# jianwen-xie/Latent-Space-Normalizing-Flow

Hardware: AMD Instinct MI355X
Metric: latent-samples/sec through flow+logdet, nz=128 B=65536 (higher is better)
Workload: dtype bf16x3; 1 GPU; CIFAR-10 flow prior nz=128 f_width=64 f_depth=5 affine, forward+logdet+log-prob, B=65536 synthetic z per evaluation (BASELINE.json configs[2]); rows_per_gpu=65536, global_rows=65536, parallelism=single GPU, streams=3, clock_ramp_launches_before_warmup=600

## Files before the change

### latent-space-normalizing-flow_amd/csrc/lsnf_fwd3p.hip

```cpp
#include <stdlib.h>
#include <type_traits>
#include "lsnf_l16.h"

#if LSNF_L16_PARTS != 3
#error "lsnf_fwd3p.hip is the three-term bf16 kernel"
#endif

#ifndef LSNF_FILLMASK
#define LSNF_FILLMASK 0x7f
#endif

namespace {

struct Fwd3pArgs {
    const float* consts; const float* panels3;
    const float* z_in; const float* objective;
    float* z_out; float* logdet_out; float* ll_out;
    int B, nz, half, n_blocks, vec4;
    double* stats;
    float* hdump; int width;
    float* z_saved; float* act_saved;
    unsigned long long* stamps;
};

#ifdef LSNF_STAMPS
#define P_STAMP(i, INSN)                                                                                \
    do { __builtin_amdgcn_sched_barrier(0);                                                             \
         unsigned long long t_; asm volatile(INSN " %0\n\ts_waitcnt lgkmcnt(0)" : "=s"(t_) :: "memory");  \
         __builtin_amdgcn_sched_barrier(0);                                                             \
         if (a.stamps && lane == 0) a.stamps[(((size_t)blockIdx.x * NWAVES + wave) & 2047) * 64 + (i)] = t_; } while (0)
#else
#define P_STAMP(i, INSN) do {} while (0)
#endif

template <int WT_>
struct Fwd3pCfg : LsnfStackCfg<2, WT_> {
    using S = LsnfStackCfg<2, WT_>;
    static constexpr int F = LSNF_FRAG3_FLOATS;
    static constexpr int OFF3_S2 = F * S::P1 * S::KT1;
    static constexpr int OFF3_S3 = OFF3_S2 + F * S::P2 * S::KT2;
    static constexpr int OFF3_S4 = OFF3_S3 + F * S::P3 * S::KT3;
    static constexpr int BLOCK3 = OFF3_S4 + F * S::P4 * S::KT4;
    static constexpr int SLOT3 = 2 * S::MAXKT * F;
    static constexpr int CONST_FLOATS = S::FWD_CONST;
};

__device__ __forceinline__ void keep(unsigned a, unsigned b, unsigned c) { asm volatile("" :: "v"(a), "v"(b), "v"(c)); }
__device__ __forceinline__ void keep(float a, float b, float c, float d, float e) { asm volatile("" :: "v"(a), "v"(b), "v"(c), "v"(d), "v"(e)); }

struct StepDesc { int acc, tile, s, frag; };
template <int KT> constexpr StepDesc mkstep(int acc, int tl, int in_tile, int kt, int s) { return StepDesc{acc, in_tile, s, ((tl * KT + kt) * 2 + s) * 3}; }

struct Tile16 { f32x4v q[4]; };
struct SplitTile16 { unsigned d[2][3][4]; };

template <int HT, int ST>
__device__ __forceinline__ Tile16 load_tile16(int t, const float* __restrict__ z, const int* rows, int nz, int half, int g, int vw) {
    Tile16 x;
    const int hh = t / HT, tt = t % HT;
#pragma unroll
    for (int ft = 0; ft < 2; ++ft)
#pragma unroll
        for (int st = 0; st < ST; ++st) {
            const int f0 = 32 * tt + l16_feat0(ft, g), col0 = hh * half + f0, q = 2 * ft + st;
            const float* zr = z + (long)rows[st] * (long)nz;
            if (vw == 4) {
                f32x4 v = {0.f, 0.f, 0.f, 0.f};
                if (f0 < half) v = *reinterpret_cast<const f32x4*>(zr + col0);
                x.q[q][0] = v[0]; x.q[q][1] = v[1]; x.q[q][2] = v[2]; x.q[q][3] = v[3];
            } else if (vw == 2) {
                f32x2 v0 = {0.f, 0.f}, v1 = {0.f, 0.f};
                if (f0 < half) v0 = *reinterpret_cast<const f32x2*>(zr + col0);
                if (f0 + 2 < half) v1 = *reinterpret_cast<const f32x2*>(zr + col0 + 2);
                x.q[q][0] = v0[0]; x.q[q][1] = v0[1]; x.q[q][2] = v1[0]; x.q[q][3] = v1[1];
            } else {
#pragma unroll
                for (int j = 0; j < 4; ++j) x.q[q][j] = (f0 + j < half) ? zr[col0 + j] : 0.0f;
            }
        }
    return x;
}
template <int HT, int ST>
__device__ __forceinline__ void store_tile16(int t, const Tile16& x, float* __restrict__ z, const int* rows, const bool* live,
                                             int nz, int half, int g, int vw) {
    const int hh = t / HT, tt = t % HT;
#pragma unroll
    for (int ft = 0; ft < 2; ++ft)
#pragma unroll
        for (int st = 0; st < ST; ++st) {
            if (!live[st]) continue;
            const int f0 = 32 * tt + l16_feat0(ft, g), col0 = hh * half + f0, q = 2 * ft + st;
            float* zr = z + (long)rows[st] * (long)nz;
            if (vw == 4) {
                if (f0 < half) { f32x4 v = {x.q[q][0], x.q[q][1], x.q[q][2], x.q[q][3]}; *reinterpret_cast<f32x4*>(zr + col0) = v; }
            } else if (vw == 2) {
                if (f0 < half) { f32x2 v = {x.q[q][0], x.q[q][1]}; *reinterpret_cast<f32x2*>(zr + col0) = v; }
                if (f0 + 2 < half) { f32x2 v = {x.q[q][2], x.q[q][3]}; *reinterpret_cast<f32x2*>(zr + col0 + 2) = v; }
            } else {
#pragma unroll
                for (int j = 0; j < 4; ++j)
                    if (f0 + j < half) zr[col0 + j] = x.q[q][j];
            }
        }
}
__device__ __forceinline__ const float* bias_lane_ptr(const float* cb, int g) { return cb + (g & 1) * 16 + 4 * (g >> 1); }
__device__ __forceinline__ f32x4v bias_quad(const float* lane_ptr, int float_off) {
    const f32x4 v = *reinterpret_cast<const f32x4*>(lane_ptr + float_off);
    f32x4v r;
#pragma unroll
    for (int j = 0; j < 4; ++j) r[j] = v[j];
    return r;
}
template <class PH> constexpr bool first_touch(int i) {
    for (int j = 0; j < i; ++j)
        if (PH::at(j).acc == PH::at(i).acc && PH::at(j).s == PH::at(i).s) return false;
    return true;
}
template <int ST> __device__ __forceinline__ constexpr int unit_quad(int q) { return ST == 2 ? q : (q & ~1); }
template <int ST> __device__ __forceinline__ constexpr int unit_pair0(int q) { return ST == 2 ? 0 : (q & 1); }
template <int ST> __device__ __forceinline__ constexpr int unit_st(int q) { return ST == 2 ? (q & 1) : 0; }
template <bool RELU, int ST>
__device__ __forceinline__ void split_q16(const Tile16& x, int q, SplitTile16& out) {
#pragma clang fp contract(off)
    const int ft = q >> 1, st = unit_st<ST>(q), qr = unit_quad<ST>(q);
#pragma unroll
    for (int jj = 0; jj < ST; ++jj) {
        const int j = unit_pair0<ST>(q) + jj;
        float a = x.q[qr][2 * j], b = x.q[qr][2 * j + 1];
        if (RELU) { a = fmaxf(a, 0.0f); b = fmaxf(b, 0.0f); }
        const unsigned p1 = pk_bf16(a, b);
        a -= __builtin_bit_cast(float, p1 << 16); b -= __builtin_bit_cast(float, p1 & 0xffff0000u);
        const unsigned p2 = pk_bf16(a, b);
        a -= __builtin_bit_cast(float, p2 << 16); b -= __builtin_bit_cast(float, p2 & 0xffff0000u);
        const int d = 2 * ft + j;
        out.d[st][0][d] = p1; out.d[st][1][d] = p2; out.d[st][2][d] = pk_bf16(a, b);
        keep(out.d[st][0][d], out.d[st][1][d], out.d[st][2][d]);
    }
}
template <int ST>
__device__ __forceinline__ void sigmoid_q16(Tile16& p, int q, float* lsum ) {
    const int st = unit_st<ST>(q), qr = unit_quad<ST>(q), r0 = 2 * unit_pair0<ST>(q);
#pragma unroll
    for (int r = r0; r < r0 + 2 * ST; ++r) {
        float sig, l2;
        lsnf_sigmoid_log2(p.q[qr][r], sig, l2);
        p.q[qr][r] = sig; lsum[st] += l2;
    }
    keep(p.q[qr][r0], p.q[qr][r0 + 1], p.q[qr][r0 + 2 * ST - 2], p.q[qr][r0 + 2 * ST - 1], lsum[st]);
}
template <int ST>
__device__ __forceinline__ void couple_q16(Tile16& v, const Tile16& t, const Tile16& sig, int q) {
    const int qr = unit_quad<ST>(q), r0 = 2 * unit_pair0<ST>(q);
#pragma unroll
    for (int r = r0; r < r0 + 2 * ST; ++r) v.q[qr][r] = (v.q[qr][r] + t.q[qr][r]) * sig.q[qr][r];
}

#ifndef LSNF_STASH_AUX
#define LSNF_STASH_AUX 0
#endif
#ifndef LSNF_STASH_PARTS
#define LSNF_STASH_PARTS 7
#endif
typedef unsigned u32x4s __attribute__((ext_vector_type(4)));
struct StashLane { unsigned zoff, soff, moff, msh, hoff; };
struct StashRsrc { __amdgpu_buffer_rsrc_t r[2]; };
__device__ __forceinline__ StashRsrc stash_rsrc(const float* p, unsigned bytes, unsigned second_off) {
    char* c = reinterpret_cast<char*>(const_cast<float*>(p));
    return StashRsrc{{__builtin_amdgcn_make_buffer_rsrc(c, 0, (int)bytes, 0x00020000),
                      __builtin_amdgcn_make_buffer_rsrc(c + second_off, 0, (int)(bytes > second_off ? bytes - second_off : 0u), 0x00020000)}};
}
template <int HT>
__device__ __forceinline__ void stash_row_quad(const StashRsrc& rs, const StashLane& sl, int t, int q, const Tile16& x, int nz, int half, int g) {
    if constexpr (!(LSNF_STASH_PARTS & 4)) return;
    const int ft = q >> 1, st = q & 1, hh = t / HT, tt = t % HT;
    unsigned off = sl.zoff;
    if (st) off += (unsigned)(16 * nz * 4);
    off = (32 * tt + 16 * ft + 4 * g < half) ? off : 0x80000000u;
    const u32x4s v = __builtin_bit_cast(u32x4s, x.q[q]);
    __builtin_amdgcn_raw_buffer_store_b128(v, rs.r[hh], off + (unsigned)((32 * tt + 16 * ft) * 4), 0, LSNF_STASH_AUX);
}
__device__ __forceinline__ void stash_sigma_quad(const StashRsrc& rs, const StashLane& sl, int t, int q, const Tile16& sg) {
    if constexpr (!(LSNF_STASH_PARTS & 2)) return;
    const int ft = q >> 1, st = q & 1;
    const u32x4s v = __builtin_bit_cast(u32x4s, sg.q[q]);
    __builtin_amdgcn_raw_buffer_store_b128(v, rs.r[t], sl.soff + (unsigned)((2 * ft * 64 + 16 * st) * 16), 0, LSNF_STASH_AUX);
}
__device__ __forceinline__ void mask_q16(const Tile16& h, int q, unsigned (&mk)[2][2]) {
    if constexpr (!(LSNF_STASH_PARTS & 1)) return;
    unsigned m = 0;
#pragma unroll
    for (int r = 3; r >= 0; --r) m = __builtin_amdgcn_alignbit(m, __builtin_bit_cast(unsigned, 0.0f - h.q[q][r]), 31);
    mk[q & 1][q >> 1] = m;
    asm volatile("" :: "v"(m));
}
__device__ __forceinline__ void stash_mask_words(const StashRsrc& rs, const StashLane& sl, int tile, const unsigned (&mk)[2][2]) {
    if constexpr (!(LSNF_STASH_PARTS & 1)) return;
    const unsigned w0 = mk[0][0] | (mk[0][1] << 8), w1 = mk[1][0] | (mk[1][1] << 8);
    unsigned x = ((w0 << 16) | w1) << sl.msh;
    x = lsnf_pair_or32(x);
    __builtin_amdgcn_raw_buffer_store_b32(x >> 16, rs.r[0], sl.moff + (unsigned)(tile * 64 * 4), 0, 0);
    __builtin_amdgcn_raw_buffer_store_b32(x & 0xffffu, rs.r[0], sl.moff + (unsigned)((tile * 64 + 16) * 4), 0, 0);
}
__device__ __forceinline__ void stash_h_quad(const StashRsrc& rs, const StashLane& sl, int t, int q, const Tile16& h, int width) {
    const int ft = q >> 1, st = q & 1;
    f32x4v r;
#pragma unroll
    for (int j = 0; j < 4; ++j) r[j] = fmaxf(h.q[q][j], 0.0f);
    const unsigned off = (32 * t + 16 * ft < width) ? sl.hoff : 0x80000000u;
    __builtin_amdgcn_raw_buffer_store_b128(__builtin_bit_cast(u32x4s, r), rs.r[t], off + (unsigned)((ft * 2 + st) * 1024), 0, LSNF_STASH_AUX);
}

template <int NM, int NV>
__device__ __forceinline__ void pin_mfma() {
    lsnf_static_for<NM>([&](auto mc) {
        constexpr int m = decltype(mc)::value, V = NV / NM + (m < NV % NM ? 1 : 0);
        __builtin_amdgcn_sched_group_barrier(0x008, 1, 0);
        if constexpr (V > 0) __builtin_amdgcn_sched_group_barrier(0x402, V, 0);
    });
}
template <class PH, int ST, class Fill, class Mid>
__device__ __forceinline__ void run_phase16(Tile16* acc, const float* bias_ptr , const SplitTile16* in, const float* lbuf, int lane, Fill&& fill, Mid&& mid) {
    const bf16x8* wp = reinterpret_cast<const bf16x8*>(lbuf) + lane;
    __builtin_amdgcn_sched_barrier(0);
    bf16x8 a[3];
#pragma unroll
    for (int p = 0; p < 3; ++p) a[p] = wp[(PH::at(0).frag + p) * 64];
    f32x4v bq = bias_quad(bias_ptr, 32 * PH::btile(PH::at(0).acc) + 8 * PH::at(0).s);
    __builtin_amdgcn_sched_group_barrier(0x100, 4, 0);
    lsnf_static_for<PH::N>([&](auto ic) {
        constexpr int i = decltype(ic)::value;
        constexpr StepDesc d = PH::at(i);
        mid(ic);
        bf16x8 na[3];
        f32x4v nbq = bq;
#pragma unroll
        for (int p = 0; p < 3; ++p) na[p] = a[p];
        if constexpr (i + 1 < PH::N) {
#pragma unroll
            for (int p = 0; p < 3; ++p) na[p] = wp[(PH::at(i + 1).frag + p) * 64];
            if constexpr (first_touch<PH>(i + 1)) nbq = bias_quad(bias_ptr, 32 * PH::btile(PH::at(i + 1).acc) + 8 * PH::at(i + 1).s);
        }
#ifndef LSNF_ABL_NOFILL
        fill(ic);
#endif
        const SplitTile16& x = in[d.tile];
        constexpr bool first = first_touch<PH>(i);
#define LSNF_Q_MMA(WI, XI) \
        acc[d.acc].q[2 * d.s + 0] = __builtin_amdgcn_mfma_f32_16x16x32_bf16(a[WI], __builtin_bit_cast(bf16x8, u32x4{x.d[0][XI][0], x.d[0][XI][1], x.d[0][XI][2], x.d[0][XI][3]}), (first && WI == 2 && XI == 0) ? bq : acc[d.acc].q[2 * d.s + 0], 0, 0, 0); \
        if constexpr (ST == 2) acc[d.acc].q[2 * d.s + 1] = __builtin_amdgcn_mfma_f32_16x16x32_bf16(a[WI], __builtin_bit_cast(bf16x8, u32x4{x.d[1][XI][0], x.d[1][XI][1], x.d[1][XI][2], x.d[1][XI][3]}), (first && WI == 2 && XI == 0) ? bq : acc[d.acc].q[2 * d.s + 1], 0, 0, 0);
#ifdef LSNF_ABL_NOMFMA
        LSNF_Q_MMA(0, 0)
#else
        LSNF_F3_TERMS(LSNF_Q_MMA)
#endif
#undef LSNF_Q_MMA
        if constexpr (i + 1 < PH::N) __builtin_amdgcn_sched_group_barrier(0x100, first_touch<PH>(i + 1) ? 4 : 3, 0);
        pin_mfma<6 * ST, (PH::valu(i) * ST) / 2>();
        __builtin_amdgcn_sched_barrier(0);
#pragma unroll
        for (int p = 0; p < 3; ++p) a[p] = na[p];
        bq = nbq;
    });
}

struct QhNoStores { static constexpr int stores(int) { return 0; } };
struct QhS1a : QhNoStores {
    static constexpr int N = 16;
    static constexpr int btile(int acc) { return acc; }
    static constexpr StepDesc at(int i) { return mkstep<4>((i >> 1) & 1, (i >> 1) & 1, i >> 2, i >> 2, i & 1); }
    static constexpr int valu(int i) { return i < 2 ? 22 : (i < 6 ? 28 : (i < 8 ? 16 : (i < 12 ? 22 : 0))); }
};
struct QhS1b : QhNoStores {
    static constexpr int N = 16;
    static constexpr int btile(int acc) { return 2 + acc; }
    static constexpr StepDesc at(int i) { return mkstep<4>((i >> 1) & 1, (i >> 1) & 1, i >> 2, i >> 2, i & 1); }
    static constexpr int valu(int i) { return i >= 8 ? 22 : 0; }
};
struct QhS23 : QhNoStores {
    static constexpr int N = 16;
    static constexpr int btile(int acc) { return 4 + acc; }
    static constexpr StepDesc at(int i) {
        if (i < 8) { const int tl = i >> 2, kt = (i >> 1) & 1; return mkstep<2>(tl, tl, kt, kt, i & 1); }
        const int j = i - 8, kt = j >> 2, tl = (j >> 1) & 1;
        return mkstep<2>(2 + tl, 2 + tl, 2 + kt, kt, j & 1);
    }
    static constexpr int valu(int i) { return (i >= 4 && i < 12) ? 26 : (i >= 13 ? 26 : 0); }
};
struct QhS4 : QhNoStores {
    static constexpr int N = 16;
    static constexpr int btile(int acc) { return 8 + (acc == 0 ? 2 : (acc == 1 ? 0 : (acc == 2 ? 3 : 1))); }
    static constexpr int torder(int j) { return j == 0 ? 2 : (j == 1 ? 0 : (j == 2 ? 3 : 1)); }
    static constexpr StepDesc at(int i) { const int kt = i >> 3, j = (i >> 1) & 3; return mkstep<2>(j, torder(j), kt, kt, i & 1); }
    static constexpr int valu(int i) { return i < 4 ? 26 : (i < 9 ? 0 : (i < 12 ? 28 : (i == 12 ? 36 : (i == 13 ? 24 : 22)))); }
};

struct QsS1a : QhS1a {
    static constexpr int valu(int i) { return (i == 6 || i == 7) ? 20 : (i >= 8 && i < 12 ? 23 : QhS1a::valu(i)); }
    static constexpr int stores(int i) { return (i >= 2 && i < 6) ? 1 : ((i == 6 || i == 7) ? 2 : (i >= 8 && i < 12 ? 1 : 0)); }
};
struct QsS1b : QhS1b {
    static constexpr int valu(int i) { return i < 8 ? (i >= 6 ? 1 : 0) : (i < 14 ? 23 : 22); }
    static constexpr int stores(int i) { return (i >= 6 && i < 14) ? 1 : 0; }
};
struct QsS23 : QhS23 {
    static constexpr int valu(int i) { return (i >= 4 && i < 12) ? (i == 8 ? 44 : 34) : (i >= 13 ? 34 : 0); }
    static constexpr int stores(int i) { return i == 8 ? 2 : 0; }
};
struct QsS4 : QhS4 {
    static constexpr int valu(int i) { return i < 4 ? 34 : ((i >= 6 && i < 9) ? 10 + QhS4::valu(i) : QhS4::valu(i)); }
    static constexpr int stores(int i) { return (i >= 6 && i < 9) ? 2 : ((i >= 9 && i < 13) ? 1 : 0); }
};
struct QxS23 : QsS23 {
    static constexpr int valu(int i) { return QsS23::valu(i) + (((i >= 4 && i < 12) || i >= 13) ? 2 : 0); }
    static constexpr int stores(int i) { return QsS23::stores(i) + (((i >= 4 && i < 12) || i >= 13) ? 1 : 0); }
};
struct QxS4 : QsS4 {
    static constexpr int valu(int i) { return QsS4::valu(i) + (i < 4 ? 2 : 0); }
    static constexpr int stores(int i) { return QsS4::stores(i) + (i < 4 ? 1 : 0); }
};
template <class PH> constexpr int stores_after(int last_dma_step) {
    int n = 0;
    for (int i = last_dma_step + 1; i < PH::N; ++i) n += PH::stores(i);
    return n;
}

template <int WT, int NWAVES, int ST, int STASH = 0>
__global__ __launch_bounds__(64 * NWAVES, 1) void lsnf_fwd3q_kernel(const Fwd3pArgs a) {
    static_assert(!STASH || ST == 2, "the stash tile is a wave's 32 rows");
    using TS1a = std::conditional_t<STASH != 0, QsS1a, QhS1a>;
    using TS1b = std::conditional_t<STASH != 0, QsS1b, QhS1b>;
    using TS23 = std::conditional_t<STASH == 2, QxS23, std::conditional_t<STASH != 0, QsS23, QhS23>>;
    using TS4 = std::conditional_t<STASH == 2, QxS4, std::conditional_t<STASH != 0, QsS4, QhS4>>;
    using C = Fwd3pCfg<WT>;
    static_assert(WT == 2, "lsnf_fwd3q_kernel: f_width <= 64 instantiation");
    constexpr int THREADS = 64 * NWAVES;
    constexpr int HT = 2, NZT = 4, F = C::F;
    constexpr int SLOT = C::SLOT3;
    extern __shared__ __attribute__((aligned(16))) float smem[];
    float* cst = smem;
    float* const buf0 = smem + a.n_blocks * C::CONST_FLOATS;
    const int tid = threadIdx.x;
    const int wave = __builtin_amdgcn_readfirstlane(tid >> 6);
    const int lane = tid & 63;
    const int n = lane & 15, g = lane >> 4;
    P_STAMP(0, "s_memtime");
    P_STAMP(50, "s_memrealtime");
    const int n_phases = 4 * a.n_blocks;
    auto phase_src = [&](int k) -> const float* {
        const float* gb = a.panels3 + (size_t)(k >> 2) * C::BLOCK3;
        const int j = k & 3;
        return gb + (j == 0 ? 0 : (j == 1 ? 2 * 4 * F : (j == 2 ? C::OFF3_S2 : C::OFF3_S4)));
    };
    auto sync_issue = [&](int k, auto left) {
#ifdef LSNF_ABL_SKIPSYNC
        if ((LSNF_ABL_SKIPSYNC >> (k & 3)) & 1) return;
#endif
        asm volatile("s_waitcnt vmcnt(%0)" :: "n"(decltype(left)::value) : "memory");
        __syncthreads();
#ifdef LSNF_FWD3Q_BURST_DMA
        if (k + 1 < n_phases) issue_kib<48, NWAVES>(phase_src(k + 1), buf0 + ((k + 1) & 1) * SLOT, wave, lane);
#endif
    };
    constexpr int PER_WAVE = 48 / NWAVES, EVERY = STASH ? 1 : 16 / PER_WAVE, LAST_DMA = (PER_WAVE - 1) * EVERY;
    using Left0 = std::integral_constant<int, 0>;
    using LeftS1a = std::integral_constant<int, stores_after<TS1a>(LAST_DMA)>;
    using LeftS1b = std::integral_constant<int, stores_after<TS1b>(LAST_DMA)>;
    using LeftS23 = std::integral_constant<int, stores_after<TS23>(LAST_DMA) + (STASH == 2 ? 1 : 0)>;
    using LeftS4 = std::integral_constant<int, stores_after<TS4>(LAST_DMA)>;
    const float* dma_src = nullptr; float* dma_dst = nullptr;
    auto dma_arm = [&](int k) {
        dma_src = phase_src(k + 1 < n_phases ? k + 1 : k);
        dma_dst = buf0 + ((k + 1) & 1) * SLOT;
    };
    auto dma_step = [&](auto ic) {
#ifndef LSNF_FWD3Q_BURST_DMA
        constexpr int i = decltype(ic)::value;
        if constexpr (i % EVERY == 0 && i / EVERY < PER_WAVE) issue_piece<NWAVES>(dma_src, dma_dst, i / EVERY, wave, lane);
#endif
    };

    const int wbase = (blockIdx.x * NWAVES + wave) * (16 * ST);
    int sample[2] = {0, 0}, rows[2] = {0, 0}; bool live[2] = {false, false};
#pragma unroll
    for (int st = 0; st < ST; ++st) { sample[st] = wbase + 16 * st + n; live[st] = sample[st] < a.B; rows[st] = live[st] ? sample[st] : a.B - 1; }

    Tile16 v[NZT];
    SplitTile16 xs[NZT];
    Tile16 p1, t1;
    float lsum[2] = {0.0f, 0.0f};
    {
        const Tile16 x0 = load_tile16<HT, ST>(0, a.z_in, rows, a.nz, a.half, g, a.vec4);
        const Tile16 x1 = load_tile16<HT, ST>(1, a.z_in, rows, a.nz, a.half, g, a.vec4);
        v[2] = load_tile16<HT, ST>(2, a.z_in, rows, a.nz, a.half, g, a.vec4);
        v[3] = load_tile16<HT, ST>(3, a.z_in, rows, a.nz, a.half, g, a.vec4);
        __builtin_amdgcn_sched_barrier(0);
        issue_kib<48, NWAVES>(phase_src(0), buf0, wave, lane);
        for (int i = tid; i < a.n_blocks * C::CONST_FLOATS; i += THREADS) cst[i] = a.consts[i];
#pragma unroll
        for (int q = 0; q < 4; ++q) { split_q16<false, ST>(x0, q, xs[0]); split_q16<false, ST>(x1, q, xs[1]); }
        split_q16<false, ST>(v[2], 0, xs[2]); split_q16<false, ST>(v[2], 1, xs[2]);
#pragma unroll
        for (int q = 0; q < 4; ++q)
#pragma unroll
            for (int r = 0; r < 4; ++r) { p1.q[q][r] = 80.0f; t1.q[q][r] = 0.0f; }
    }
    float ell[2];
#pragma unroll
    for (int st = 0; st < 2; ++st) ell[st] = (st < ST && a.objective) ? a.objective[rows[st]] : 0.0f;
    float ss01[2] = {0.0f, 0.0f};
    StashLane sl0 = {0u, 0u, 0u, 0u};
    const LsnfActLayout al = lsnf_act_layout(a.B, HT, WT);
    const unsigned zbytes = (unsigned)a.B * (unsigned)a.nz * 4u, abytes = (unsigned)(al.per_block * 4);
    if constexpr (STASH) {
        const unsigned tile_byte = (unsigned)(wbase >> 5) * (unsigned)(al.per_tile * 4), L = (unsigned)(n + 32 * (g & 1));
        sl0.zoff = ((unsigned)(wbase + n) * (unsigned)a.nz + 4u * g) * 4u;
        sl0.soff = tile_byte + ((unsigned)(g >> 1) * 64u + L) * 16u;
        sl0.moff = tile_byte + (unsigned)(al.mask_off * 4) + L * 4u;
        sl0.msh = 4u * (g >> 1);
        sl0.hoff = (unsigned)(wbase >> 5) * (unsigned)(32 * a.width * 4) + (unsigned)(n * 4 + g) * 16u;
    }
    const LsnfDumpLayout dl = lsnf_dump_layout(a.B, a.nz, a.width);
    const unsigned hbytes = (unsigned)(((size_t)a.B + 31) / 32 * 32 * a.width * 4);
    sync_issue(0, Left0{});
    P_STAMP(1, "s_memtime");

    for (int blk = 0; blk < a.n_blocks; ++blk) {
        const float* cb = cst + blk * C::CONST_FLOATS;
        const bool more = blk + 1 < a.n_blocks;
        const int k0 = 4 * blk;
        SplitTile16 vh[4];
        SplitTile16 h2s[WT];
        Tile16 hh[4], tp[4];
        const bool zs = STASH && a.z_saved != nullptr, as = STASH && a.act_saved != nullptr;
        const float* zc = more ? (zs ? a.z_saved + (size_t)blk * a.B * a.nz : a.z_out) : a.z_out;
        const float* zp = blk > 0 ? (zs ? a.z_saved + (size_t)(blk - 1) * a.B * a.nz : a.z_out) : a.z_out;
        const StashRsrc rs_zc = stash_rsrc(zc, (more && !zs) ? 0u : zbytes, (unsigned)a.half * 4u);
        const StashRsrc rs_zp = stash_rsrc(zp, (blk > 0 && !zs) ? 0u : zbytes, (unsigned)a.half * 4u);
        const StashRsrc rs_ac = stash_rsrc(as ? a.act_saved + (size_t)blk * al.per_block : a.z_out, as ? abytes : 0u, 4096u);
        const StashRsrc rs_ap = stash_rsrc(as ? a.act_saved + (size_t)(blk > 0 ? blk - 1 : 0) * al.per_block : a.z_out, as ? abytes : 0u, 4096u);
        StashLane sl = sl0;
        if constexpr (STASH) asm volatile("" : "+v"(sl.zoff), "+v"(sl.soff), "+v"(sl.moff));
        if constexpr (STASH == 2) asm volatile("" : "+v"(sl.hoff));
        const float* hd = (STASH == 2) ? a.hdump + (size_t)blk * dl.per_block : a.z_out;
        const StashRsrc rs_h1 = stash_rsrc(STASH == 2 ? hd + dl.off_h1 : hd, STASH == 2 ? hbytes : 0u, 4096u);
        const StashRsrc rs_h2 = stash_rsrc(STASH == 2 ? hd + dl.off_h2 : hd, STASH == 2 ? hbytes : 0u, 4096u);
        unsigned mk1[2][2], mk2[2][2], mk3[2][2];

        if (blk == 1) P_STAMP(10, "s_memtime");
        {
            const float* bv = bias_lane_ptr(cb, g);
            if (k0 > 0) sync_issue(k0, LeftS4{});
            dma_arm(k0);
            run_phase16<TS1a, ST>(v, bv, xs, buf0 + (k0 & 1) * SLOT, lane, [&](auto ic) {
                constexpr int i = decltype(ic)::value;
                if constexpr (STASH && i >= 8 && i < 12) stash_row_quad<HT>(rs_zp, sl, 2, i - 8, v[2], a.nz, a.half, g);
                if constexpr (i < 2) split_q16<false, ST>(v[2], 2 + i, xs[2]);
                else if constexpr (i < 6) {
                    sigmoid_q16<ST>(p1, i - 2, lsum);
                    if constexpr (STASH) stash_sigma_quad(rs_ap, sl, 1, i - 2, p1);
                } else if constexpr (i < 8) {
                    couple_q16<ST>(v[3], t1, p1, 2 * (i - 6)); couple_q16<ST>(v[3], t1, p1, 2 * (i - 6) + 1);
                    if constexpr (STASH) { stash_row_quad<HT>(rs_zp, sl, 3, 2 * (i - 6), v[3], a.nz, a.half, g); stash_row_quad<HT>(rs_zp, sl, 3, 2 * (i - 6) + 1, v[3], a.nz, a.half, g); }
                } else if constexpr (i < 12) split_q16<false, ST>(v[3], i - 8, xs[3]);
            }, dma_step);
        }
        if (blk == 1) P_STAMP(11, "s_memtime");
        {
            const float* bv = bias_lane_ptr(cb, g);
            sync_issue(k0 + 1, LeftS1a{});
            dma_arm(k0 + 1);
            run_phase16<TS1b, ST>(v + 2, bv, xs, buf0 + ((k0 + 1) & 1) * SLOT, lane, [&](auto ic) {
                constexpr int i = decltype(ic)::value;
                if constexpr (STASH && i >= 6 && i < 14) stash_row_quad<HT>(rs_zc, sl, (i - 6) >> 2, (i - 6) & 3, v[(i - 6) >> 2], a.nz, a.half, g);
                if constexpr (i >= 8) split_q16<false, ST>(v[(i - 8) >> 2], i & 3, vh[(i - 8) >> 2]);
            }, dma_step);
        }
        if (blk == 1) P_STAMP(12, "s_memtime");
        if (!more) {
            int ln = lane;
            asm volatile("" : "+v"(ln));
            const int smp[2] = {wbase + (ln & 15), wbase + 16 + (ln & 15)};
#pragma unroll
            for (int t = 0; t < HT; ++t) {
                if constexpr (!STASH) store_tile16<HT, ST>(t, v[t], a.z_out, smp, live, a.nz, a.half, g, a.vec4);
#pragma unroll
                for (int ft = 0; ft < 2; ++ft)
#pragma unroll
                    for (int st = 0; st < ST; ++st)
#pragma unroll
                        for (int r = 0; r < 4; ++r) ss01[st] += v[t].q[2 * ft + st][r] * v[t].q[2 * ft + st][r];
            }
        }
#pragma unroll
        for (int st = 0; st < 2; ++st) { ell[st] = ell[st] + cb[32 * C::NP + 0]; ell[st] = ell[st] + cb[32 * C::NP + 1]; }
        {
            static_assert(C::P1 == 4 && C::P2 == 2 && C::P3 == 2, "bias tile indices of the phase tables");
            const float* bv = bias_lane_ptr(cb, g);
            sync_issue(k0 + 2, LeftS1b{});
            dma_arm(k0 + 2);
            run_phase16<TS23, ST>(hh, bv, vh, buf0 + ((k0 + 2) & 1) * SLOT, lane, [&](auto ic) {
                constexpr int i = decltype(ic)::value;
                if constexpr (i >= 4 && i < 8) split_q16<true, ST>(hh[0], i - 4, vh[2]);
                if constexpr (i >= 8 && i < 12) split_q16<true, ST>(hh[1], i - 8, vh[3]);
                if constexpr (i >= 13) split_q16<true, ST>(hh[2], i - 13, h2s[0]);
                if constexpr (STASH) {
                    if constexpr (i >= 4 && i < 8) mask_q16(hh[0], i - 4, mk3);
                    if constexpr (i == 8) stash_mask_words(rs_ac, sl, 0, mk3);
                    if constexpr (i >= 8 && i < 12) mask_q16(hh[1], i - 8, mk1);
                    if constexpr (i >= 13) mask_q16(hh[2], i - 13, mk2);
                }
                if constexpr (STASH == 2) {
                    if constexpr (i >= 4 && i < 8) stash_h_quad(rs_h1, sl, 0, i - 4, hh[0], a.width);
                    if constexpr (i >= 8 && i < 12) stash_h_quad(rs_h1, sl, 1, i - 8, hh[1], a.width);
                    if constexpr (i >= 13) stash_h_quad(rs_h2, sl, 0, i - 13, hh[2], a.width);
                }
            }, dma_step);
        }
        if (blk == 1) P_STAMP(13, "s_memtime");
        xs[0] = vh[0]; xs[1] = vh[1];
        {
            constexpr int B4 = C::P1 + C::P2 + C::P3;
            static_assert(B4 == 8, "bias tile indices of the phase tables");
            const float* bv = bias_lane_ptr(cb, g);
            split_q16<true, ST>(hh[2], 3, h2s[0]);
            if constexpr (STASH) mask_q16(hh[2], 3, mk2);
            if constexpr (STASH == 2) stash_h_quad(rs_h2, sl, 0, 3, hh[2], a.width);
            sync_issue(k0 + 3, LeftS23{});
            dma_arm(k0 + 3);
            run_phase16<TS4, ST>(tp, bv, h2s, buf0 + ((k0 + 3) & 1) * SLOT, lane, [&](auto ic) {
                constexpr int i = decltype(ic)::value;
                if constexpr (i < 4) split_q16<true, ST>(hh[3], i, h2s[1]);
                if constexpr (STASH) {
                    if constexpr (i < 4) mask_q16(hh[3], i, mk3);
                    if constexpr (i == 6) stash_mask_words(rs_ac, sl, 1, mk1);
                    if constexpr (i == 7) stash_mask_words(rs_ac, sl, WT + 0, mk2);
                    if constexpr (i == 8) stash_mask_words(rs_ac, sl, WT + 1, mk3);
                }
                if constexpr (STASH == 2 && i < 4) stash_h_quad(rs_h2, sl, 1, i, hh[3], a.width);
                if constexpr (i >= 9 && i < 13) { sigmoid_q16<ST>(tp[0], i - 9, lsum); if constexpr (STASH) stash_sigma_quad(rs_ac, sl, 0, i - 9, tp[0]); }
                if constexpr (i == 12) couple_q16<ST>(v[2], tp[1], tp[0], 0);
                if constexpr (i == 13) { couple_q16<ST>(v[2], tp[1], tp[0], 1); couple_q16<ST>(v[2], tp[1], tp[0], 2); couple_q16<ST>(v[2], tp[1], tp[0], 3); }
                if constexpr (i >= 14) split_q16<false, ST>(v[2], i - 14, xs[2]);
            }, dma_step);
            p1 = tp[2]; t1 = tp[3];
        }
        if (blk == 1) P_STAMP(14, "s_memtime");
    }
    P_STAMP(40, "s_memtime");
#pragma unroll
    for (int q = 0; q < 4; ++q) { sigmoid_q16<ST>(p1, q, lsum); couple_q16<ST>(v[3], t1, p1, q); }
    if constexpr (STASH) {
        const bool as = a.act_saved != nullptr;
        const StashRsrc rs_al = stash_rsrc(as ? a.act_saved + (size_t)(a.n_blocks - 1) * al.per_block : a.z_out, as ? abytes : 0u, 4096u);
#pragma unroll
        for (int q = 0; q < 4; ++q) stash_sigma_quad(rs_al, sl0, 1, q, p1);
    }
#pragma unroll
    for (int st = 0; st < ST; ++st) ell[st] = ell[st] + -0.6931471805599453f * l16_group_sum(lsum[st]);

    float ss[2] = {ss01[0], ss01[1]};
    int ln_e = lane;
    asm volatile("" : "+v"(ln_e));
    const int smp_e[2] = {wbase + (ln_e & 15), wbase + 16 + (ln_e & 15)};
#pragma unroll
    for (int t = HT; t < NZT; ++t) {
#pragma unroll
        for (int ft = 0; ft < 2; ++ft)
#pragma unroll
            for (int st = 0; st < ST; ++st)
#pragma unroll
                for (int r = 0; r < 4; ++r) ss[st] += v[t].q[2 * ft + st][r] * v[t].q[2 * ft + st][r];
        store_tile16<HT, ST>(t, v[t], a.z_out, smp_e, live, a.nz, a.half, g, a.vec4);
    }
    float ll[2] = {0.0f, 0.0f};
#pragma unroll
    for (int st = 0; st < ST; ++st) {
        ll[st] = (-0.5f * l16_group_sum(ss[st]) + 1.8378770664093453f) + ell[st];
        if (live[st] && g == 0) {
            const int smp = smp_e[st];
            a.logdet_out[smp] = ell[st];
            if (a.ll_out) a.ll_out[smp] = ll[st];
        }
    }
    asm volatile("s_waitcnt vmcnt(0)" ::: "memory");
    if (a.stats) {
        double dl = 0.0, dd = 0.0;
#pragma unroll
        for (int st = 0; st < ST; ++st)
            if (live[st] && g == 0) { dl += (double)ll[st]; dd += (double)ell[st]; }
#pragma unroll
        for (int o = 8; o > 0; o >>= 1) { dl += __shfl_xor(dl, o, 64); dd += __shfl_xor(dd, o, 64); }
        __syncthreads();
        double* red = reinterpret_cast<double*>(buf0);
        if (lane == 0) { red[2 * wave] = dl; red[2 * wave + 1] = dd; }
        __syncthreads();
        if (wave == 0) {
            double tl = 0.0, td = 0.0;
            for (int w = 0; w < NWAVES; ++w) { tl += red[2 * w]; td += red[2 * w + 1]; }
            lsnf_publish_stats(a.stats, tl, td, a.B, lane);
        }
    }
    P_STAMP(41, "s_memtime");
    P_STAMP(51, "s_memrealtime");
}

size_t fwd3q_lds(int n_blocks) {
    using C = Fwd3pCfg<2>;
    return ((size_t)n_blocks * C::CONST_FLOATS + 2 * (size_t)C::SLOT3) * sizeof(float);
}

template <int WT, int NWAVES, int ST, int STASH = 0>
hipError_t launch_fwd3q_w(const Fwd3pArgs& a, hipStream_t stream) {
    const size_t lds = fwd3q_lds(a.n_blocks);
    auto kern = lsnf_fwd3q_kernel<WT, NWAVES, ST, STASH>;
    static unsigned long long lds_ok = 0;
    if (hipError_t e = lsnf_allow_big_lds((const void*)kern, &lds_ok); e != hipSuccess) return e;
    const unsigned grid = (unsigned)((a.B + 16 * ST * NWAVES - 1) / (16 * ST * NWAVES));
    hipLaunchKernelGGL(kern, dim3(grid), dim3(64 * NWAVES), lds, stream, a);
    return hipGetLastError();
}
}

bool lsnf_forward3q_covers(const LsnfGeo& g, int first_block, int n_blocks, int B, int vec4, const float* z_out,
                           const float* z_saved, const float* act_saved, const float* hdump, int hdump_tiled) {
    if (g.HT != 2 || g.WT != 2 || fwd3q_lds(n_blocks) > 160 * 1024) return false;
    if (hdump && (!hdump_tiled || !act_saved || (n_blocks > 1 && !z_saved) || first_block != 0 || (g.width & 15) ||
                  ((size_t)B + 32) * g.width * 4 >= (1ull << 31))) return false;
    const bool stash = act_saved != nullptr || z_saved != nullptr;
    return !(stash && (vec4 != 4 || (size_t)B * g.nz * 4 >= (1ull << 31) || lsnf_act_layout(B, g.HT, g.WT).per_block * 4 >= (1ull << 31) ||
                       (((size_t)act_saved | (size_t)z_saved | (size_t)z_out) & 15)));
}

hipError_t lsnf_launch_forward3q(const LsnfGeo& g, const float* plan, int first_block, int n_blocks, int B,
                                 const float* z_in, const float* objective, float* z_out, float* logdet_out,
                                 float* ll_out, float* z_saved, float* act_saved, double* stats, int vec4, hipStream_t stream,
                                 float* hdump, int hdump_tiled) {
    if (!lsnf_forward3q_covers(g, first_block, n_blocks, B, vec4, z_out, z_saved, act_saved, hdump, hdump_tiled))
        return hipErrorInvalidValue;
    const bool stash = act_saved != nullptr || z_saved != nullptr;
    Fwd3pArgs a;
    a.consts = plan + g.off_fwd_const + (size_t)first_block * g.fwd_const_floats;
    a.panels3 = plan + g.off_f3b_panels + (size_t)first_block * g.f3_block_floats;
    a.z_in = z_in; a.objective = objective; a.z_out = z_out; a.logdet_out = logdet_out; a.ll_out = ll_out;
    a.B = B; a.nz = g.nz; a.half = g.half; a.n_blocks = n_blocks; a.vec4 = vec4; a.stats = stats;
    a.z_saved = z_saved; a.act_saved = act_saved ? act_saved + (size_t)first_block * lsnf_act_layout(B, g.HT, g.WT).per_block : nullptr;
    a.hdump = hdump; a.width = g.width;
    a.stamps = lsnf_stamps_buffer();
    static const char* shape = getenv("LSNF_FWD3Q_SHAPE");
    const int sh = shape ? atoi(shape) : (B > 128 * 256 ? 82 : (B > 64 * 256 ? 81 : 41));
    if (hdump) return (sh == 82) ? launch_fwd3q_w<2, 8, 2, 2>(a, stream) : launch_fwd3q_w<2, 4, 2, 2>(a, stream);
    if (stash) return (sh == 82) ? launch_fwd3q_w<2, 8, 2, 1>(a, stream) : launch_fwd3q_w<2, 4, 2, 1>(a, stream);
    if (sh == 82) return launch_fwd3q_w<2, 8, 2>(a, stream);
    if (sh == 42) return launch_fwd3q_w<2, 4, 2>(a, stream);
    if (sh == 81) return launch_fwd3q_w<2, 8, 1>(a, stream);
    return launch_fwd3q_w<2, 4, 1>(a, stream);
}
```

Before: 761.7 million latent-samples/s.

## Reorder S23 MFMA steps so ReLU splits finish inside the phase, not after

Reorders the second and third layer MFMA step sequence in the non-stash S23 phase so each hidden tile completes earlier. Its ReLU/bf16 split work can then start sooner and the last h2 quad no longer spills past the phase boundary. The stash variant keeps the old k-major order through a new QhS23Kmajor table. ReLU is also rewritten as fmed3 with an SGPR infinity. This is meant to allow source-modifier folding and to cut VALU work.

```diff
diff --git a/latent-space-normalizing-flow_amd/csrc/lsnf_fwd3p.hip b/latent-space-normalizing-flow_amd/csrc/lsnf_fwd3p.hip
--- a/latent-space-normalizing-flow_amd/csrc/lsnf_fwd3p.hip
+++ b/latent-space-normalizing-flow_amd/csrc/lsnf_fwd3p.hip
@@ -119,6 +119,11 @@
 template <int ST> __device__ __forceinline__ constexpr int unit_quad(int q) { return ST == 2 ? q : (q & ~1); }
 template <int ST> __device__ __forceinline__ constexpr int unit_pair0(int q) { return ST == 2 ? 0 : (q & 1); }
 template <int ST> __device__ __forceinline__ constexpr int unit_st(int q) { return ST == 2 ? (q & 1) : 0; }
+__device__ __forceinline__ float relu_mfma(float h) {
+    float inf = __builtin_inff();
+    asm("" : "+s"(inf));
+    return __builtin_amdgcn_fmed3f(h, 0.0f, inf);
+}
 template <bool RELU, int ST>
 __device__ __forceinline__ void split_q16(const Tile16& x, int q, SplitTile16& out) {
 #pragma clang fp contract(off)
@@ -127,7 +132,7 @@
     for (int jj = 0; jj < ST; ++jj) {
         const int j = unit_pair0<ST>(q) + jj;
         float a = x.q[qr][2 * j], b = x.q[qr][2 * j + 1];
-        if (RELU) { a = fmaxf(a, 0.0f); b = fmaxf(b, 0.0f); }
+        if (RELU) { a = relu_mfma(a); b = relu_mfma(b); }
         const unsigned p1 = pk_bf16(a, b);
         a -= __builtin_bit_cast(float, p1 << 16); b -= __builtin_bit_cast(float, p1 & 0xffff0000u);
         const unsigned p2 = pk_bf16(a, b);
@@ -205,7 +210,7 @@
     const int ft = q >> 1, st = q & 1;
     f32x4v r;
 #pragma unroll
-    for (int j = 0; j < 4; ++j) r[j] = fmaxf(h.q[q][j], 0.0f);
+    for (int j = 0; j < 4; ++j) r[j] = relu_mfma(h.q[q][j]);
     const unsigned off = (32 * t + 16 * ft < width) ? sl.hoff : 0x80000000u;
     __builtin_amdgcn_raw_buffer_store_b128(__builtin_bit_cast(u32x4s, r), rs.r[t], off + (unsigned)((ft * 2 + st) * 1024), 0, LSNF_STASH_AUX);
 }
@@ -277,14 +282,24 @@
     static constexpr int valu(int i) { return i >= 8 ? 22 : 0; }
 };
 struct QhS23 : QhNoStores {
-    static constexpr int N = 16;
+    static constexpr int N = 16, H10 = 2, H11 = 6, H20 = 12;
+    static constexpr int btile(int acc) { return 4 + acc; }
+    static constexpr int s3(int j) { return j == 0 ? 0 : (j == 1 ? 2 : (j == 2 ? 4 : (j == 3 ? 1 : (j == 4 ? 3 : (j == 5 ? 6 : (j == 6 ? 5 : 7)))))); }
+    static constexpr StepDesc at(int i) {
+        if (i < 8) { const int tl = i >> 2, ft = (i >> 1) & 1, kt = i & 1; return mkstep<2>(tl, tl, kt, kt, ft); }
+        const int c = s3(i - 8), tl = c >> 2, ft = (c >> 1) & 1, kt = c & 1;
+        return mkstep<2>(2 + tl, 2 + tl, 2 + kt, kt, ft);
+    }
+    static constexpr int valu(int i) { return (i >= 2 && i < 10) || i >= 12 ? 26 : 0; }
+};
+struct QhS23Kmajor : QhNoStores {
+    static constexpr int N = 16, H10 = 4, H11 = 8, H20 = 13, MW = 8;
     static constexpr int btile(int acc) { return 4 + acc; }
     static constexpr StepDesc at(int i) {
         if (i < 8) { const int tl = i >> 2, kt = (i >> 1) & 1; return mkstep<2>(tl, tl, kt, kt, i & 1); }
         const int j = i - 8, kt = j >> 2, tl = (j >> 1) & 1;
         return mkstep<2>(2 + tl, 2 + tl, 2 + kt, kt, j & 1);
     }
-    static constexpr int valu(int i) { return (i >= 4 && i < 12) ? 26 : (i >= 13 ? 26 : 0); }
 };
 struct QhS4 : QhNoStores {
     static constexpr int N = 16;
@@ -302,7 +317,7 @@
     static constexpr int valu(int i) { return i < 8 ? (i >= 6 ? 1 : 0) : (i < 14 ? 23 : 22); }
     static constexpr int stores(int i) { return (i >= 6 && i < 14) ? 1 : 0; }
 };
-struct QsS23 : QhS23 {
+struct QsS23 : QhS23Kmajor {
     static constexpr int valu(int i) { return (i >= 4 && i < 12) ? (i == 8 ? 44 : 34) : (i >= 13 ? 34 : 0); }
     static constexpr int stores(int i) { return i == 8 ? 2 : 0; }
 };
@@ -365,7 +380,8 @@
     using Left0 = std::integral_constant<int, 0>;
     using LeftS1a = std::integral_constant<int, stores_after<TS1a>(LAST_DMA)>;
     using LeftS1b = std::integral_constant<int, stores_after<TS1b>(LAST_DMA)>;
-    using LeftS23 = std::integral_constant<int, stores_after<TS23>(LAST_DMA) + (STASH == 2 ? 1 : 0)>;
+    constexpr bool H2_EXPOSED = TS23::H20 + 4 > TS23::N;
+    using LeftS23 = std::integral_constant<int, stores_after<TS23>(LAST_DMA) + (STASH == 2 && H2_EXPOSED ? 1 : 0)>;
     using LeftS4 = std::integral_constant<int, stores_after<TS4>(LAST_DMA)>;
     const float* dma_src = nullptr; float* dma_dst = nullptr;
     auto dma_arm = [&](int k) {
@@ -500,19 +516,20 @@
             dma_arm(k0 + 2);
             run_phase16<TS23, ST>(hh, bv, vh, buf0 + ((k0 + 2) & 1) * SLOT, lane, [&](auto ic) {
                 constexpr int i = decltype(ic)::value;
-                if constexpr (i >= 4 && i < 8) split_q16<true, ST>(hh[0], i - 4, vh[2]);
-                if constexpr (i >= 8 && i < 12) split_q16<true, ST>(hh[1], i - 8, vh[3]);
-                if constexpr (i >= 13) split_q16<true, ST>(hh[2], i - 13, h2s[0]);
+                constexpr int H10 = TS23::H10, H11 = TS23::H11, H20 = TS23::H20;
+                if constexpr (i >= H10 && i < H10 + 4) split_q16<true, ST>(hh[0], i - H10, vh[2]);
+                if constexpr (i >= H11 && i < H11 + 4) split_q16<true, ST>(hh[1], i - H11, vh[3]);
+                if constexpr (i >= H20) split_q16<true, ST>(hh[2], i - H20, h2s[0]);
                 if constexpr (STASH) {
-                    if constexpr (i >= 4 && i < 8) mask_q16(hh[0], i - 4, mk3);
-                    if constexpr (i == 8) stash_mask_words(rs_ac, sl, 0, mk3);
-                    if constexpr (i >= 8 && i < 12) mask_q16(hh[1], i - 8, mk1);
-                    if constexpr (i >= 13) mask_q16(hh[2], i - 13, mk2);
+                    if constexpr (i >= H10 && i < H10 + 4) mask_q16(hh[0], i - H10, mk3);
+                    if constexpr (i == TS23::MW) stash_mask_words(rs_ac, sl, 0, mk3);
+                    if constexpr (i >= H11 && i < H11 + 4) mask_q16(hh[1], i - H11, mk1);
+                    if constexpr (i >= H20) mask_q16(hh[2], i - H20, mk2);
                 }
                 if constexpr (STASH == 2) {
-                    if constexpr (i >= 4 && i < 8) stash_h_quad(rs_h1, sl, 0, i - 4, hh[0], a.width);
-                    if constexpr (i >= 8 && i < 12) stash_h_quad(rs_h1, sl, 1, i - 8, hh[1], a.width);
-                    if constexpr (i >= 13) stash_h_quad(rs_h2, sl, 0, i - 13, hh[2], a.width);
+                    if constexpr (i >= H10 && i < H10 + 4) stash_h_quad(rs_h1, sl, 0, i - H10, hh[0], a.width);
+                    if constexpr (i >= H11 && i < H11 + 4) stash_h_quad(rs_h1, sl, 1, i - H11, hh[1], a.width);
+                    if constexpr (i >= H20) stash_h_quad(rs_h2, sl, 0, i - H20, hh[2], a.width);
                 }
             }, dma_step);
         }
@@ -522,9 +539,11 @@
             constexpr int B4 = C::P1 + C::P2 + C::P3;
             static_assert(B4 == 8, "bias tile indices of the phase tables");
             const float* bv = bias_lane_ptr(cb, g);
-            split_q16<true, ST>(hh[2], 3, h2s[0]);
-            if constexpr (STASH) mask_q16(hh[2], 3, mk2);
-            if constexpr (STASH == 2) stash_h_quad(rs_h2, sl, 0, 3, hh[2], a.width);
+            if constexpr (H2_EXPOSED) {
+                split_q16<true, ST>(hh[2], 3, h2s[0]);
+                if constexpr (STASH) mask_q16(hh[2], 3, mk2);
+                if constexpr (STASH == 2) stash_h_quad(rs_h2, sl, 0, 3, hh[2], a.width);
+            }
             sync_issue(k0 + 3, LeftS23{});
             dma_arm(k0 + 3);
             run_phase16<TS4, ST>(tp, bv, h2s, buf0 + ((k0 + 3) & 1) * SLOT, lane, [&](auto ic) {
```

Result: faster. 771.3 million latent-samples/s, median of 6 (+1.3%).
